# metacraft-labs/dvt-circuits

Hardware: AMD Instinct MI355X
Metric: SP1 prover cycles/sec + proofs/hour, finalization_prove at 1/2/4/8 MI355X (higher is better)
Workload: dtype u32; 1 GPU; BASELINE configs[1] input: examples/finalization_test.json (tests/golden/finalization_example.json) through the reference's JSON -> CBOR -> SP1Stdin encoding, executed AND proven (the whole prove() call) by the finalization-shaped synthetic guest tests/guests.py:dkg_like(6180, 1545, 1): 32 shards of 2^21 RV32IM cycles; the reference's own guest ELF is prebuilt machine code and is not run (it would; stdin_bytes=2165, participants=3, curve_precompiles=False, fri_queries=100, pow_bits=16, log_blowup=1

## Files before the change

### dvt_circuits_amd/capi.py

```python
import ctypes as C
import json
import os
import subprocess

import numpy as np

HERE = os.path.dirname(os.path.abspath(__file__))
LIB_PATH = os.path.join(HERE, "libdvt_prover.so")
CSRC = os.path.join(HERE, "csrc")

DVT_OK, DVT_ERR_GUEST, DVT_ERR_INPUT, DVT_ERR_DEVICE, DVT_ERR_UNSUPPORTED, DVT_ERR_REJECTED = 0, 1, 2, 3, 4, 5
PATHS = {"default": 0, "rows": 1, "parts": 2}
SELECTORS = {"table": 0, "kernel": 1}
DVT_KEEP_NONE, DVT_KEEP_TREE, DVT_KEEP_FULL = 0, 1, 2
u32p = C.POINTER(C.c_uint32)
u8p = C.POINTER(C.c_uint8)


class DevMatrix(C.Structure):
    _fields_ = [("d_data", C.c_void_p), ("width", C.c_uint32), ("log_height", C.c_uint32)]


class HostTrace(C.Structure):
    _fields_ = [("chip_id", C.c_uint32), ("log_n", C.c_uint32), ("data", u32p)]
# ... 86 lines not shown
    lib.dvt_stage_hunt_join_free.argtypes = [vp, vp]
    lib.dvt_rv32_hunt_join_job.argtypes = [vp, vp, vp, C.POINTER(JoinWindow), sz, u32p, u32, u64, u32p, u32, u32p, u32p, u64, sz, sz, u32,
                                           C.POINTER(JoinSummary), C.POINTER(JoinCell), sz, C.POINTER(sz), C.POINTER(JoinCell), sz, C.POINTER(sz)]
    lib.dvt_rv32_job_shard_chips.argtypes = [vp, sz]
    lib.dvt_rv32_job_shard_chips.restype = u32
    lib.dvt_rv32_job_shard_chip_shape.argtypes = [vp, sz, u32, u32p, u32p]
    lib.dvt_machine_setup.argtypes = [vp, C.c_char_p, C.POINTER(HostTrace), sz, C.POINTER(vp), C.POINTER(u8p), C.POINTER(sz)]
    lib.dvt_pk_free.argtypes = [vp, vp]
    lib.dvt_pk_free.restype = None
    lib.dvt_machine_prove.argtypes = [vp, vp, C.POINTER(HostTrace), sz, u32p, sz, C.POINTER(u8p), C.POINTER(sz)]
    lib.dvt_machine_verify.argtypes = [C.c_char_p, sz, C.c_char_p, sz, u32, u32, C.POINTER(C.c_char_p)]
    lib.dvt_prover_machine_verify.argtypes = [vp, C.c_char_p, sz, C.c_char_p, sz, u32, u32, C.POINTER(C.c_char_p)]
    lib.dvt_prover_verify.argtypes = [vp, C.c_char_p, sz, C.c_char_p, sz, u32, u32, C.POINTER(C.c_int32), C.POINTER(u8p), C.POINTER(sz), C.POINTER(C.c_char_p)]
    lib.dvt_prover_verify_times.argtypes = [vp, C.POINTER(C.c_double)]
    lib.dvt_stage_sponge_rows.argtypes = [vp, u32p, u32p, sz, u32p]
    lib.dvt_stage_verify_paths.argtypes = [vp, C.POINTER(PathChain), sz, u8p]
    lib.dvt_stage_multipath_nodes.argtypes = [u32, u32p, sz, u32p, sz, C.POINTER(sz)]
    lib.dvt_stage_verify_multipath.argtypes = [vp, u32, u32p, u32p, sz, u8p, u32p, u32p, sz, u32p, u8p]
    for fn in (lib.dvt_proof_compact, lib.dvt_proof_expand):
        fn.argtypes = [C.c_char_p, sz, C.c_char_p, sz, u32, u32, C.POINTER(u8p), C.POINTER(sz), C.POINTER(C.c_char_p)]
    lib.dvt_debug_compact_list_sweep.argtypes = [C.c_char_p, sz, C.c_char_p, sz, u32, u32, C.POINTER(u64), C.POINTER(u64), C.POINTER(C.c_char_p)]
    lib.dvt_last_stage_ms.argtypes = [vp, C.POINTER(C.c_float)]
    lib.dvt_setup.argtypes = [vp, C.c_char_p, sz, C.POINTER(vp), C.POINTER(u8p), C.POINTER(sz)]
    lib.dvt_execute.argtypes = [C.c_char_p, sz, C.POINTER(Buf), sz, C.c_uint64, C.POINTER(u8p), C.POINTER(sz), C.POINTER(Report), C.POINTER(C.c_char_p)]
    lib.dvt_execute_io.argtypes = [C.c_char_p, sz, C.POINTER(Buf), sz, C.c_uint64, C.POINTER(u8p), C.POINTER(sz), C.POINTER(u8p), C.POINTER(sz), C.POINTER(Report), C.POINTER(C.c_char_p)]
    lib.dvt_debug_exec_rate.argtypes = [C.c_char_p, sz, C.POINTER(Buf), sz, u32, C.c_int]
    lib.dvt_debug_exec_rate.restype = C.c_double
    lib.dvt_debug_p2_f64_selfcheck.argtypes = [u32, u32]
    lib.dvt_debug_p2_f64_selfcheck.restype = u64
    lib.dvt_debug_p2_f64_sbox_check.argtypes = [u32, u32, C.POINTER(C.c_double)]
    lib.dvt_debug_p2_f64_sbox_check.restype = u64
    lib.dvt_debug_ntt_group_check.argtypes = [u32, u32] + [C.POINTER(C.c_double)] * 3
    lib.dvt_debug_ntt_group_check.restype = u64
    lib.dvt_prove_core.argtypes = [vp, vp, C.POINTER(Buf), sz, C.POINTER(u8p), C.POINTER(sz), C.POINTER(Report)]
    lib.dvt_verify.argtypes = [C.c_char_p, sz, C.c_char_p, sz, u32, u32, C.POINTER(C.c_int32), C.POINTER(u8p), C.POINTER(sz), C.POINTER(C.c_char_p)]
    lib.dvt_rv32_prepare.argtypes = [vp, vp, C.POINTER(Buf), sz, C.POINTER(vp), C.POINTER(Report)]
    lib.dvt_rv32_prepare_part.argtypes = [vp, vp, C.POINTER(Buf), sz, sz, sz, C.POINTER(vp), C.POINTER(Report)]
    lib.dvt_rv32_header_words.restype = u32
    lib.dvt_rv32_job_exec_wait_seconds.argtypes = [vp]
    lib.dvt_rv32_job_exec_wait_seconds.restype = C.c_double
    lib.dvt_rv32_prove_job.argtypes = [vp, vp, vp, C.POINTER(u8p), C.POINTER(sz)]
    lib.dvt_job_free.argtypes = [vp, vp]
    lib.dvt_job_free.restype = None
    lib.dvt_rv32_debug_traces.argtypes = [C.c_char_p, sz, C.POINTER(Buf), sz, u32, u32, u32p, C.POINTER(u32p), C.POINTER(sz), C.POINTER(C.c_char_p)]
    lib.dvt_rv32_job_shards.argtypes = [vp]
    lib.dvt_rv32_job_shards.restype = sz
    lib.dvt_rv32_job_shard_member.argtypes = [vp, sz]
    lib.dvt_rv32_job_shard_member.restype = C.c_int
    lib.dvt_rv32_job_shard_device_rows.argtypes = [vp, sz]
    lib.dvt_rv32_job_shard_device_rows.restype = u32
    lib.dvt_rv32_job_shard_kept.argtypes = [vp, sz]
    lib.dvt_rv32_job_shard_kept.restype = C.c_int
    lib.dvt_rv32_job_shard_kept_bytes.argtypes = [vp, sz]
    lib.dvt_rv32_job_shard_kept_bytes.restype = C.c_uint64
    lib.dvt_debug_keep_plan.argtypes = [C.c_int, u64, u64, u64, u64, u64, u64, u64, C.c_int, C.c_int64, u64]
    lib.dvt_debug_keep_plan.restype = C.c_int
    lib.dvt_rv32_commit_shard.argtypes = [vp, vp, vp, sz, u32p]
    lib.dvt_rv32_challenges.argtypes = [C.c_char_p, sz, u32p, sz, u32p]
    lib.dvt_rv32_prove_shard.argtypes = [vp, vp, vp, sz, u32p, C.POINTER(u8p), C.POINTER(sz)]
    lib.dvt_rv32_assemble.argtypes = [vp, C.POINTER(C.c_char_p), C.POINTER(sz), sz, C.POINTER(u8p), C.POINTER(sz)]
    lib.dvt_rv32_debug_device_traces.argtypes = [vp, vp, vp, sz, C.POINTER(u32p), C.POINTER(sz)]
    lib.dvt_rv32_debug_poke_cell.argtypes = [vp, vp, sz, u32, u32, u32, u32]
    prof_out = [C.POINTER(u64), sz, C.POINTER(ProfileEdge), sz, C.POINTER(ProfileSyscall), sz, C.POINTER(ProfileOpcode), sz, C.POINTER(ProfileSummary)]
    lib.dvt_rv32_job_profile.argtypes = [vp, vp, vp, u32] + prof_out
    lib.dvt_execute_profile.argtypes = [C.c_char_p, sz, C.POINTER(Buf), sz, u64] + prof_out + [C.POINTER(Report), C.POINTER(C.c_char_p)]
    tree_out = [C.POINTER(CalltreeArc), sz, C.POINTER(CalltreeFunc), sz, C.POINTER(CalltreeSummary)]
# ... 629 lines not shown
                    max_cycles=0, log_shard=21):
    lib = load()
    reps, err = (Report(), Report()), C.c_char_p()
    a, b = bytes(stdin_a), bytes(stdin_b)
    rc, got = _diverge(lambda *io: lib.dvt_execute_diverge(elf, len(elf), a, len(a), b, len(b), max_cycles, log_shard, *io, C.byref(reps[0]), C.byref(reps[1]),
                                                           C.byref(err)), start_a, start_b, max_pairs, rejoin, window, keep)
    return rc, tuple(dict(cycles=r.cycles, exit_code=r.exit_code, halted=bool(r.halted), unprovable=bool(r.unprovable)) for r in reps), got, _take_str(lib, err)


def exec_rate(elf: bytes, stdin=(), log_shard=21, trace=False) -> float:
    return float(load().dvt_debug_exec_rate(elf, len(elf), _bufs(stdin), len(stdin), log_shard, int(trace)))


def keep_plan(mode, free, total, reserve, full, tree, later, remaining=0, count_known=True, full_cap=-1, full_kept=0) -> int:
    return int(load().dvt_debug_keep_plan(mode, free, total, reserve, full, tree, later, remaining, int(bool(count_known)), full_cap, full_kept))


def p2_f64_selfcheck(n: int, seed: int) -> int:
    return int(load().dvt_debug_p2_f64_selfcheck(n, seed))


def p2_f64_sbox_check(n: int, seed: int):
    mx = (C.c_double * 4)()
    bad = load().dvt_debug_p2_f64_sbox_check(n, seed, mx)
    return int(bad), [float(v) for v in mx]


def ntt_group_check(n: int, seed: int):
    mx = [(C.c_double * 8)() for _ in range(3)]
    bad = load().dvt_debug_ntt_group_check(n, seed, *mx)
    return int(bad), {k: [float(v) for v in m] for k, m in zip(("dif", "dif_unit", "dit"), mx)}


def execute_io(elf: bytes, stdin=(), max_cycles=0):
    lib = load()
    pv, n, so, m, rep, err = u8p(), C.c_size_t(), u8p(), C.c_size_t(), Report(), C.c_char_p()
    rc = lib.dvt_execute_io(elf, len(elf), _bufs(stdin), len(stdin), max_cycles, C.byref(pv), C.byref(n), C.byref(so), C.byref(m), C.byref(rep), C.byref(err))
    out = C.string_at(pv, n.value) if pv else b""
    sout = C.string_at(so, m.value) if so else b""
    for ptr in (pv, so):
        if ptr:
            lib.dvt_free(C.cast(ptr, C.c_void_p))
    return rc, dict(cycles=rep.cycles, exit_code=rep.exit_code, halted=bool(rep.halted), unprovable=bool(rep.unprovable)), out, sout, _take_str(lib, err)


def stdin_from_json(circuit_type: str, json_bytes: bytes, auth_commitment=False) -> bytes:
    lib = load()
    out, n, err = u8p(), C.c_size_t(), C.c_char_p()
    rc = lib.dvt_stdin_from_json(circuit_type.encode(), json_bytes, len(json_bytes), int(bool(auth_commitment)), C.byref(out), C.byref(n), C.byref(err))
    if rc:
        raise DvtError(rc, _take_str(lib, err))
    b = C.string_at(out, n.value)
    lib.dvt_free(C.cast(out, C.c_void_p))
    return b


def verify(vk: bytes, proof: bytes, fri_queries=100, pow_bits=16):
    lib = load()
    ec, pv, n, why = C.c_int32(), u8p(), C.c_size_t(), C.c_char_p()
    rc = lib.dvt_verify(vk, len(vk), proof, len(proof), fri_queries, pow_bits, C.byref(ec), C.byref(pv), C.byref(n), C.byref(why))
    out = C.string_at(pv, n.value) if pv else b""
    if pv:
        lib.dvt_free(C.cast(pv, C.c_void_p))
    return rc == DVT_OK, ec.value, out, _take_str(lib, why)


# ... 658 lines not shown
```

### dvt_circuits_amd/csrc/bb.cuh

```cuda
#pragma once
#include <stdint.h>

#if defined(__HIPCC__)
#include <hip/hip_runtime.h>
#if defined(__HIP_DEVICE_COMPILE__)
#define DVT_HD __host__ __device__ __forceinline__
#else
#define DVT_HD __host__ __device__ inline
#endif
#else
#define DVT_HD inline
#endif

namespace dvt {

constexpr uint32_t P = 0x78000001u;
constexpr uint32_t MONTY_MU = 0x88000001u;
constexpr uint32_t MONTY_R = 0x0ffffffeu;
constexpr uint32_t MONTY_R2 = 0x45dddde3u;
static_assert((uint32_t)(P * MONTY_MU) == 1u, "mu");
static_assert(((uint64_t)1 << 32) % P == MONTY_R, "R");
static_assert((((uint64_t)MONTY_R * MONTY_R) % P) == MONTY_R2, "R2");

DVT_HD uint32_t mulhi_u32(uint32_t a, uint32_t b) {
// ... 67 lines not shown
    Fp c[4];
    DVT_HD static Fp4 zero() { Fp4 r; r.c[0] = r.c[1] = r.c[2] = r.c[3] = Fp::zero(); return r; }
    DVT_HD static Fp4 one() { Fp4 r = zero(); r.c[0] = Fp::one(); return r; }
    DVT_HD static Fp4 from_base(Fp a) { Fp4 r = zero(); r.c[0] = a; return r; }
    DVT_HD bool operator==(const Fp4 &o) const { return c[0] == o.c[0] && c[1] == o.c[1] && c[2] == o.c[2] && c[3] == o.c[3]; }
    DVT_HD bool operator!=(const Fp4 &o) const { return !(*this == o); }
};
DVT_HD Fp mul11(Fp a) {
    Fp a2 = dbl(a), a4 = dbl(a2), a8 = dbl(a4);
    return a8 + a2 + a;
}
DVT_HD Fp4 operator+(const Fp4 &a, const Fp4 &b) { Fp4 r; for (int i = 0; i < 4; i++) r.c[i] = a.c[i] + b.c[i]; return r; }
DVT_HD Fp4 operator-(const Fp4 &a, const Fp4 &b) { Fp4 r; for (int i = 0; i < 4; i++) r.c[i] = a.c[i] - b.c[i]; return r; }
DVT_HD Fp4 operator-(const Fp4 &a) { Fp4 r; for (int i = 0; i < 4; i++) r.c[i] = -a.c[i]; return r; }
DVT_HD Fp4 operator+(const Fp4 &a, Fp b) { Fp4 r = a; r.c[0] = r.c[0] + b; return r; }
DVT_HD Fp4 operator-(const Fp4 &a, Fp b) { Fp4 r = a; r.c[0] = r.c[0] - b; return r; }
DVT_HD Fp4 operator*(const Fp4 &a, Fp b) { Fp4 r; for (int i = 0; i < 4; i++) r.c[i] = a.c[i] * b; return r; }
DVT_HD Fp4 operator*(const Fp4 &a, const Fp4 &b) {
    Fp4 r;
    r.c[0] = a.c[0] * b.c[0] + mul11(a.c[1] * b.c[3] + a.c[2] * b.c[2] + a.c[3] * b.c[1]);
    r.c[1] = a.c[0] * b.c[1] + a.c[1] * b.c[0] + mul11(a.c[2] * b.c[3] + a.c[3] * b.c[2]);
    r.c[2] = a.c[0] * b.c[2] + a.c[1] * b.c[1] + a.c[2] * b.c[0] + mul11(a.c[3] * b.c[3]);
    r.c[3] = a.c[0] * b.c[3] + a.c[1] * b.c[2] + a.c[2] * b.c[1] + a.c[3] * b.c[0];
    return r;
}
DVT_HD Fp4 &operator+=(Fp4 &a, const Fp4 &b) { a = a + b; return a; }
DVT_HD Fp4 &operator-=(Fp4 &a, const Fp4 &b) { a = a - b; return a; }
DVT_HD Fp4 &operator*=(Fp4 &a, const Fp4 &b) { a = a * b; return a; }
DVT_HD Fp4 pow(Fp4 a, uint64_t e) {
    Fp4 r = Fp4::one();
    while (e) { if (e & 1) r = r * a; a = a * a; e >>= 1; }
    return r;
}
DVT_HD Fp4 inv(const Fp4 &a) {
    Fp A0 = a.c[0], A1 = a.c[2], B0 = a.c[1], B1 = a.c[3];
    Fp A2_0 = A0 * A0 + mul11(A1 * A1), A2_1 = dbl(A0 * A1);
    Fp B2_0 = B0 * B0 + mul11(B1 * B1), B2_1 = dbl(B0 * B1);
    Fp D0 = A2_0 - mul11(B2_1), D1 = A2_1 - B2_0;
    Fp ni = inv(D0 * D0 - mul11(D1 * D1));
    Fp I0 = D0 * ni, I1 = -(D1 * ni);
    Fp4 r;
    r.c[0] = A0 * I0 + mul11(A1 * I1);
    r.c[2] = A0 * I1 + A1 * I0;
    r.c[1] = -(B0 * I0 + mul11(B1 * I1));
    r.c[3] = -(B0 * I1 + B1 * I0);
    return r;
}

}
```

### dvt_circuits_amd/csrc/capi_rv32.hip

```cpp
#include <algorithm>
#include <atomic>
#include <cstdio>
#include <deque>
#include <map>

#include "capi_job.h"
#include "ntt_group.cuh"
#include "poseidon2_f64.cuh"
#include "sha256.h"

using namespace dvt;
static_assert(DVT_KEEP_NONE == KEEP_NONE && DVT_KEEP_TREE == KEEP_TREE && DVT_KEEP_FULL == KEEP_FULL, "the tiers of include/dvt_prover.h");

namespace {
std::vector<std::vector<uint8_t>> collect_stdin(const dvt_buf *bufs, size_t n) {
    std::vector<std::vector<uint8_t>> v(n);
    for (size_t i = 0; i < n; i++)
        if (bufs[i].len) v[i].assign(bufs[i].data, bufs[i].data + bufs[i].len);
    return v;
}
uint8_t *dup_bytes(const std::vector<uint8_t> &v, size_t *len) {
    uint8_t *b = (uint8_t *)malloc(v.size() + 1);
    if (b && !v.empty()) memcpy(b, v.data(), v.size());
    if (len) *len = v.size();
// ... 1541 lines not shown
uint64_t dvt_debug_ntt_group_check(uint32_t n, uint32_t seed, double *max_dif, double *max_dif_unit, double *max_dit) {
    uint64_t bad = 0, s = 0x9e3779b97f4a7c15ull ^ seed;
    double mx[3][8] = {};
    const int64_t lim[3] = {(int64_t)ntg::DIF_IN, (int64_t)ntg::DIF_IN, (int64_t)ntg::DIT_IN}, half = ((int64_t)P - 1) / 2;
    auto next = [&]() { s ^= s << 13; s ^= s >> 7; s ^= s << 17; return s; };
    auto uniform = [&](int64_t m) { return (int64_t)(next() % (2 * (uint64_t)m + 1)) - m; };
    int64_t in[8], tw[7];
    for (uint32_t g = 0; g < n; g++)
        for (int kind = 0; kind < 3; kind++) {
            for (int j = 0; j < 8; j++) in[j] = uniform(lim[kind]);
            for (int k = 0; k < 7; k++) tw[k] = uniform(half);
            bad += ntg_check_one(kind, in, tw, mx[kind]);
        }
    const int64_t mags[5] = {0, 1, half, (int64_t)P - 1, (int64_t)(0.52 * p2f::PD)};
    const int64_t tws[4] = {1, -1, half, -half};
    for (int kind = 0; kind < 3; kind++)
        for (int m = 0; m < 5; m++)
            for (int signs = 0; signs < 256; signs++) {
                if (m == 0 && signs) break;
                const int64_t mag = mags[m] > lim[kind] ? lim[kind] : mags[m];
                for (int j = 0; j < 8; j++) in[j] = (signs >> j) & 1 ? -mag : mag;
                for (int c = 0; c < 64 + 8; c++) {
                    for (int k = 0; k < 7; k++) {
                        const int stage = kind == 2 ? (k < 1 ? 0 : k < 3 ? 1 : 2) : (k < 4 ? 0 : k < 6 ? 1 : 2);
                        tw[k] = c < 64 ? tws[(c >> (2 * stage)) & 3] : uniform(half);
                    }
                    bad += ntg_check_one(kind, in, tw, mx[kind]);
                }
            }
    for (int k = 0; k < 8; k++) { max_dif[k] = mx[0][k]; max_dif_unit[k] = mx[1][k]; max_dit[k] = mx[2][k]; }
    return bad;
}

}
```

### dvt_circuits_amd/csrc/fri.hip

```cpp
#include "kernels.h"
#include "poseidon2_f64.cuh"
#include "f64dot.cuh"

namespace dvt {

__device__ __forceinline__ Fp root_pow24f(const NttTables &t, uint32_t e) {
    return Fp::raw(t.tw_hi[e >> 12]) * Fp::raw(t.tw_lo[e & 4095]);
}
__device__ __forceinline__ Fp4 load_ext(const Fp4 *p) {
    uint4 v = *reinterpret_cast<const uint4 *>(p);
    Fp4 r;
    r.c[0] = Fp::raw(v.x); r.c[1] = Fp::raw(v.y); r.c[2] = Fp::raw(v.z); r.c[3] = Fp::raw(v.w);
    return r;
}
__device__ __forceinline__ void store_ext(Fp4 *p, const Fp4 &v) {
    *reinterpret_cast<uint4 *>(p) = make_uint4(v.c[0].v, v.c[1].v, v.c[2].v, v.c[3].v);
}

constexpr int SCAN_PER_THREAD = 8, SCAN_BLOCK = 256 * SCAN_PER_THREAD;

__global__ void __launch_bounds__(256) scan_blocks_kernel(uint32_t *data, size_t n, uint32_t *block_sums, size_t nblocks) {
    __shared__ uint32_t wsum[256];
    uint32_t *col = data + (size_t)blockIdx.y * n;
    size_t base = (size_t)blockIdx.x * SCAN_BLOCK + (size_t)threadIdx.x * SCAN_PER_THREAD;
// ... 37 lines not shown
hipError_t launch_prefix_sum_columns(hipStream_t st, uint32_t *d_cols, uint32_t ncols, size_t n, uint32_t *d_scratch) {
    size_t nblocks = (n + SCAN_BLOCK - 1) / SCAN_BLOCK;
    dim3 grid((unsigned)nblocks, ncols);
    scan_blocks_kernel<<<grid, 256, 0, st>>>(d_cols, n, d_scratch, nblocks);
    if (nblocks > 1) {
        scan_sums_kernel<<<1, ncols, 0, st>>>(d_scratch, nblocks);
        scan_add_kernel<<<grid, 256, 0, st>>>(d_cols, n, d_scratch, nblocks);
    }
    return hipGetLastError();
}
size_t prefix_sum_scratch_words(uint32_t ncols, size_t n) { return ncols * ((n + SCAN_BLOCK - 1) / SCAN_BLOCK); }

__global__ void __launch_bounds__(256) phi_from_prefix_sums_kernel(const uint32_t *tot, uint32_t *phi, size_t n, Fp n_inv, uint32_t *cum_out) {
    size_t r = (size_t)blockIdx.x * blockDim.x + threadIdx.x;
    if (r >= n) return;
    if (r == n - 1 && cum_out) {
#pragma unroll
        for (int k = 0; k < 4; k++) cum_out[k] = tot[(size_t)k * n + n - 1];
    }
    const Fp rf = Fp::from_canonical((uint32_t)r) * n_inv;
#pragma unroll
    for (int k = 0; k < 4; k++) {
        const Fp c = Fp::raw(tot[(size_t)k * n + n - 1]) * rf;
        const Fp before = r ? Fp::raw(tot[(size_t)k * n + r - 1]) : Fp::zero();
        phi[(size_t)k * n + r] = (before - c).v;
    }
}
hipError_t launch_phi_from_prefix_sums(hipStream_t st, const uint32_t *d_totals, uint32_t *d_phi, uint32_t log_n, uint32_t *cum_out) {
    const size_t n = (size_t)1 << log_n;
    phi_from_prefix_sums_kernel<<<(unsigned)((n + 255) / 256), 256, 0, st>>>(d_totals, d_phi, n, inv(Fp::from_canonical((uint32_t)n)), cum_out);
    return hipGetLastError();
}

__global__ void __launch_bounds__(256) open_weights_kernel(Fp4 z, uint32_t log_n, Fp4 *w, NttTables tabs) {
    size_t i = (size_t)blockIdx.x * blockDim.x + threadIdx.x;
    if (i >= ((size_t)1 << log_n)) return;
    Fp x = root_pow24f(tabs, (uint32_t)i << (24 - log_n));
    Fp4 d = z - x;
    Fp4 r = inv(d) * x;
#pragma unroll
    for (int k = 0; k < 4; k++) {
        const uint32_t c = r.c[k].canonical();
        r.c[k] = Fp::raw(c > P / 2 ? c - P : c);
    }
    store_ext(w + i, r);
}
hipError_t launch_open_weights(hipStream_t st, const NttTables &tabs, Fp4 z, uint32_t log_n, Fp4 *d_w) {
    size_t n = (size_t)1 << log_n;
    open_weights_kernel<<<(unsigned)((n + 255) / 256), 256, 0, st>>>(z, log_n, d_w, tabs);
    return hipGetLastError();
}

constexpr int OPEN_CT = 4;
__global__ void __launch_bounds__(256) open_columns_kernel(const uint32_t *const *cols, uint32_t ncols, uint32_t log_n,
                                                          const Fp4 *w, Fp4 *partial) {
    __shared__ uint32_t red[256 * 4];
    const size_t n = (size_t)1 << log_n;
    const uint32_t c0 = blockIdx.y * OPEN_CT;
    DotAcc acc_l[OPEN_CT][4], acc_n[OPEN_CT][4];
#pragma unroll
    for (int c = 0; c < OPEN_CT; c++)
#pragma unroll
        for (int k = 0; k < 4; k++) acc_l[c][k] = acc_n[c][k] = DotAcc{0.0, 0.0};
    const size_t stride = (size_t)gridDim.x * 256;
    size_t i = (size_t)blockIdx.x * 256 + threadIdx.x;
    Fp4 wl, wn;
    uint32_t v[OPEN_CT];
    auto fetch = [&](size_t row) {
        wl = load_ext(w + row);
        wn = load_ext(w + ((row + n - 1) & (n - 1)));
#pragma unroll
        for (int c = 0; c < OPEN_CT; c++) v[c] = c0 + c < ncols ? cols[c0 + c][row] : 0u;
    };
    if (i < n) fetch(i);
    for (uint32_t it = 0; i < n; i += stride, it++) {
        double dl[4], dn[4], vlo[OPEN_CT], vhi[OPEN_CT];
#pragma unroll
        for (int k = 0; k < 4; k++) { dl[k] = (double)(int32_t)wl.c[k].v; dn[k] = (double)(int32_t)wn.c[k].v; }
#pragma unroll
        for (int c = 0; c < OPEN_CT; c++) { vlo[c] = (double)(v[c] & 0xffffu); vhi[c] = (double)(v[c] >> 16); }
        if (i + stride < n) fetch(i + stride);
#pragma unroll
// ... 74 lines not shown
            uint32_t v[8];
#pragma unroll
            for (int u = 0; u < 8; u++) v[u] = a.cols[c + u][i];
#pragma unroll
            for (int u = 0; u < 8; u++) {
                const double vlo = (double)(v[u] & 0xffffu), vhi = (double)(v[u] >> 16);
#pragma unroll
                for (int k = 0; k < 4; k++) acc[k].add(a.alpha_pows[4 * (c + u) + k], vlo, vhi);
            }
            if (((c - from) & 8) != 0)
#pragma unroll
                for (int k = 0; k < 4; k++) acc[k].reduce();
        }
#pragma unroll
        for (int k = 0; k < 4; k++) acc[k].reduce();
        for (; c < to; c++) {
            const uint32_t v = a.cols[c][i];
            const double vlo = (double)(v & 0xffffu), vhi = (double)(v >> 16);
#pragma unroll
            for (int k = 0; k < 4; k++) acc[k].add(a.alpha_pows[4 * c + k], vlo, vhi);
        }
#pragma unroll
        for (int k = 0; k < 4; k++) acc[k].reduce();
    };
    sweep(0, a.n_two);
#pragma unroll
    for (int k = 0; k < 4; k++) s_two.c[k] = acc[k].value();
    sweep(a.n_two, a.n_all);
    Fp4 s;
#pragma unroll
    for (int k = 0; k < 4; k++) s.c[k] = acc[k].value();
    if (a.n_two == a.n_all) s_two = s;
    Fp x = Fp::raw(a.tabs.sh_lo[1]) * root_pow24f(a.tabs, (uint32_t)i << (24 - a.log_m));
    Fp4 r = (s - a.sz_all) * inv(Fp4::from_base(x) - a.zeta);
    if (a.n_two) r += a.alpha_shift * ((s_two - a.sz_two) * inv(Fp4::from_base(x) - a.zeta_next));
    store_ext(a.out + i, r);
}
hipError_t launch_reduced_opening(hipStream_t st, const NttTables &tabs, const uint32_t *const *d_cols, uint32_t n_two,
                                  uint32_t n_all, uint32_t log_m, const double *d_alpha_pows_f64, Fp4 sz_all, Fp4 sz_two, Fp4 zeta,
                                  Fp4 zeta_next, Fp4 alpha_shift, Fp4 *d_out) {
    ReducedArgs a{d_cols, n_two, n_all, log_m, d_alpha_pows_f64, sz_all, sz_two, zeta, zeta_next, alpha_shift, d_out, tabs};
    size_t m = (size_t)1 << log_m;
    reduced_opening_kernel<<<(unsigned)((m + 255) / 256), 256, 0, st>>>(a);
    return hipGetLastError();
}

__global__ void __launch_bounds__(256) fri_fold_kernel(const Fp4 *v, Fp4 *out, const Fp4 *ro, Fp4 beta, const Fp4 *beta_dev,
                                                      uint32_t log_m, Fp inv2, NttTables tabs) {
    const size_t half = (size_t)1 << (log_m - 1);
    size_t i = (size_t)blockIdx.x * blockDim.x + threadIdx.x;
    if (i >= half) return;
    if (beta_dev) beta = load_ext(beta_dev);
    Fp4 lo = load_ext(v + i), hi = load_ext(v + i + half);
    Fp xinv = i ? root_pow24f(tabs, (uint32_t)(2 * half - i) << (24 - log_m)) : Fp::one();
    Fp4 r = (lo + hi) * inv2 + beta * ((lo - hi) * (inv2 * xinv));
    if (ro) r += load_ext(ro + i);
    store_ext(out + i, r);
}
hipError_t launch_fri_fold(hipStream_t st, const NttTables &tabs, const Fp4 *d_v, Fp4 *d_out, const Fp4 *d_ro, Fp4 beta,
                           uint32_t log_m, const Fp4 *d_beta) {
    size_t half = (size_t)1 << (log_m - 1);
    Fp inv2 = inv(Fp::two());
    fri_fold_kernel<<<(unsigned)((half + 255) / 256), 256, 0, st>>>(d_v, d_out, d_ro, beta, d_beta, log_m, inv2, tabs);
    return hipGetLastError();
}
__global__ void __launch_bounds__(64) fri_challenge_kernel(const uint32_t *root, uint32_t *state, Fp4 *beta_out, uint32_t *root_out) {
    const uint32_t e = threadIdx.x & 15;
    const p2f::CoopConsts k = p2f::coop_consts(e);
// ... 111 lines not shown
```

### dvt_circuits_amd/csrc/kernels.h

```cpp
#pragma once
#include <hip/hip_runtime.h>

#include <algorithm>
#include <cstddef>
#include <cstdint>
#include <vector>

#include "bb.cuh"
#include "poseidon2.cuh"

namespace dvt {

constexpr uint32_t LDE_MAX_LOG = 23;
struct NttTables {
    uint32_t *base = nullptr;
    const uint32_t *tw_hi = nullptr, *tw_lo = nullptr, *sh_hi = nullptr, *sh_lo = nullptr;
    const uint32_t *lde_tw = nullptr, *lde_scale = nullptr;
    const uint32_t *lde_tw_c = nullptr, *lde_scale_c = nullptr;
};
hipError_t ntt_tables_create(NttTables *t);
void ntt_tables_destroy(NttTables *t);

hipError_t launch_coset_lde(hipStream_t st, const NttTables &tabs, uint32_t *d_in, uint32_t *d_scratch, uint32_t *d_out,
                            uint32_t width, uint32_t log_n, uint32_t shift_mode);
hipError_t launch_to_internal(hipStream_t st, uint32_t *d, size_t n);
hipError_t launch_from_internal(hipStream_t st, uint32_t *d, size_t n);

constexpr uint32_t MERKLE_TOP_LOG = 6;
constexpr uint32_t MERKLE_COOP_LOG = 13;
constexpr uint32_t MERKLE_MAX_SEGMENTS = 24;
struct MerkleLeafSegments {
    uint32_t n = 0;
    const uint32_t *const *cols[MERKLE_MAX_SEGMENTS];
    uint32_t *out[MERKLE_MAX_SEGMENTS];
    uint32_t ncols[MERKLE_MAX_SEGMENTS], log_h[MERKLE_MAX_SEGMENTS];
    uint32_t coop[MERKLE_MAX_SEGMENTS];
    uint32_t block0[MERKLE_MAX_SEGMENTS + 1];
    void add(const uint32_t *const *c, uint32_t nc, uint32_t lh, uint32_t *o) { cols[n] = c; ncols[n] = nc; log_h[n] = lh; out[n] = o; n++; }
};
hipError_t launch_merkle_leaves(hipStream_t st, MerkleLeafSegments sg);
hipError_t launch_merkle_level(hipStream_t st, const uint32_t *d_prev, const uint32_t *d_inject, uint32_t log_len, uint32_t *d_out);
struct MerkleTopInject {
    const uint32_t *digests[MERKLE_TOP_LOG + 1] = {};
};
hipError_t launch_merkle_top(hipStream_t st, uint32_t *d_layer, uint32_t log_start, const MerkleTopInject &inj);
hipError_t launch_poseidon2_permute(hipStream_t st, uint32_t *d_states, size_t n);

hipError_t launch_prefix_sum_columns(hipStream_t st, uint32_t *d_cols, uint32_t ncols, size_t n, uint32_t *d_scratch);
size_t prefix_sum_scratch_words(uint32_t ncols, size_t n);
hipError_t launch_phi_from_prefix_sums(hipStream_t st, const uint32_t *d_totals, uint32_t *d_phi, uint32_t log_n, uint32_t *cum_out);
hipError_t launch_open_weights(hipStream_t st, const NttTables &tabs, Fp4 z, uint32_t log_n, Fp4 *d_w);
constexpr uint32_t OPEN_MAX_ROW_BLOCKS = 256;
uint32_t open_row_blocks(uint32_t log_n);
hipError_t launch_open_columns(hipStream_t st, const uint32_t *const *d_cols, uint32_t ncols, uint32_t log_n, const Fp4 *d_w,
                               Fp4 *d_partial, Fp4 *d_out);
hipError_t launch_reduced_opening(hipStream_t st, const NttTables &tabs, const uint32_t *const *d_cols, uint32_t n_two,
                                  uint32_t n_all, uint32_t log_m, const double *d_alpha_pows_f64, Fp4 sz_all, Fp4 sz_two, Fp4 zeta,
                                  Fp4 zeta_next, Fp4 alpha_shift, Fp4 *d_out);
hipError_t launch_fri_fold(hipStream_t st, const NttTables &tabs, const Fp4 *d_v, Fp4 *d_out, const Fp4 *d_ro, Fp4 beta,
                           uint32_t log_m, const Fp4 *d_beta = nullptr);
hipError_t launch_fri_challenge(hipStream_t st, const uint32_t *d_root, uint32_t *d_state, Fp4 *d_beta_out, uint32_t *d_root_out);
hipError_t launch_fri_leaves(hipStream_t st, const Fp4 *d_v, uint32_t log_m, uint32_t *d_digests);
hipError_t launch_gather_rows(hipStream_t st, const uint32_t *const *d_cols, const uint32_t *d_log_h, uint32_t ncols,
                              const uint32_t *d_idx, uint32_t nq, uint32_t *d_out);
hipError_t launch_gather_paths(hipStream_t st, const uint32_t *d_digests, uint32_t log_h, const uint32_t *d_idx, uint32_t nq,
                               uint32_t *d_out);
hipError_t launch_gather_nodes(hipStream_t st, const uint32_t *d_digests, const uint32_t *d_at, uint32_t n, uint32_t *d_out);
hipError_t launch_gather_siblings(hipStream_t st, const Fp4 *d_v, uint32_t log_m, const uint32_t *d_idx, uint32_t nq, Fp4 *d_out);
hipError_t launch_pow_grind(hipStream_t st, const uint32_t state[16], uint32_t pos, uint32_t bits, uint32_t base, uint32_t count,
                            uint32_t *d_found);


namespace rv32 { struct CycleRec; }
enum ProfileCounter { PROFILE_TRANSFERS, PROFILE_DROPPED, PROFILE_SYS_OVERFLOW, PROFILE_BAD_RECORDS, PROFILE_COUNTERS };
struct ProfileTables {
    unsigned long long *pc_count, *taken;
    unsigned long long *edge_keys, *edge_counts;
    unsigned long long *sys_keys, *sys_counts;
    unsigned long long *counters;
    const uint32_t *classes;
    uint32_t n_instr, log_slots;
};
hipError_t launch_profile_records(hipStream_t st, const rv32::CycleRec *d_recs, size_t n_recs, uint32_t last_succ, const ProfileTables &t);
// ... 87 lines not shown
```

### dvt_circuits_amd/csrc/machine_rv32.hip

```cpp
#include "machine.h"
#if !defined(__HIP_DEVICE_COMPILE__)
#pragma clang optimize off
#endif
#include "gen/air_rv32.inc"
#if !defined(__HIP_DEVICE_COMPILE__)
#pragma clang optimize on
#endif

namespace dvt {
ChipDesc rv32_wide_chip_desc(int chip);
void rv32_check_fns(int chip, ChipDesc *d);
void rv32_wide_check_fns(int chip, ChipDesc *d);
void rv32_ledger_fns(int chip, ChipDesc *d);
void rv32_wide_ledger_fns(int chip, ChipDesc *d);
void rv32_hunt_fns(int chip, ChipDesc *d);
void rv32_wide_hunt_fns(int chip, ChipDesc *d);
void rv32_join_fns(int chip, ChipDesc *d);
void rv32_wide_join_fns(int chip, ChipDesc *d);
namespace {
template <int I, class A>
ChipDesc chip_desc_here() {
    ChipDesc d;
    if constexpr (I < RV32_FIRST_WIDE_CHIP) { d = make_chip_desc<A>(); rv32_check_fns(I, &d); rv32_ledger_fns(I, &d); rv32_hunt_fns(I, &d); rv32_join_fns(I, &d); }
    else { d = rv32_wide_chip_desc(I); rv32_wide_check_fns(I, &d); rv32_wide_ledger_fns(I, &d); rv32_wide_hunt_fns(I, &d); rv32_wide_join_fns(I, &d); }
    return d;
}
}
#define DVT_X(i, A) chip_desc_here<i, A>(),
static const ChipDesc rv32_chips[] = {DVT_AIR_RV32_CHIPS(DVT_X)};
#undef DVT_X
static const MachineDesc rv32_machine = {"rv32", air_rv32::N_CHIPS, rv32_chips};
const MachineDesc *machine_rv32() { return &rv32_machine; }
}
```

### dvt_circuits_amd/csrc/stark.cuh

```cuda
#pragma once
#include "bb.cuh"
#include "f64dot.cuh"
#include "kernels.h"

namespace dvt {

constexpr int WHEN_ALL = 0, WHEN_FIRST = 1, WHEN_LAST = 2, WHEN_TRANS = 3;

DVT_HD Fp4 to_ext(Fp a) { return Fp4::from_base(a); }
DVT_HD Fp4 to_ext(const Fp4 &a) { return a; }

template <class Air>
struct PermShape {
    static constexpr int NB = (Air::N_INTERACTIONS + 1) / 2;
    static constexpr int EXT_W = Air::N_INTERACTIONS ? NB : 0;
    static constexpr int PHI = NB - 1;
    static constexpr int BASE_W = 4 * EXT_W;
    static constexpr int N_FOLDED = Air::N_CONSTRAINTS + (Air::N_INTERACTIONS ? NB : 0);
};

template <class Air, class TT, class Access>
struct ConstraintFolder {
    using T = TT;
    using Shape = PermShape<Air>;
// ... 147 lines not shown
            Air::interactions(*this);
        } else if constexpr (PART < Air::N_PARTS) {
            Air::template constraints_part<PART>(*this);
        } else {
            Air::template interactions_part<PART - Air::N_PARTS>(*this);
        }
        if constexpr (BASE) {
            acc += acc_d.value();
            Fp4 lc;
            for (int k = 0; k < 4; k++) lc.c[k] = Fp::raw(p2f::to_mont(acc_c.c[k]));
            acc += lc;
        }
        return acc;
    }
};

#if defined(__HIPCC__)
struct PermArgs {
    const uint32_t *main;
    const uint32_t *prep;
    const uint32_t *pub;
    uint32_t *perm;
    uint32_t *totals;
    const Fp4 *beta_pows;
    const double *beta_d;
    Fp4 perm_alpha;
    uint32_t log_n;
    uint32_t *partial = nullptr;
};
constexpr int PARTS_MAX = 32;
constexpr uint32_t PARTS_PARALLEL_LOG = 15;

template <class Air>
struct PermRowCtx {
    using T = Fp;
    const PermArgs &a;
    size_t n, row;
    Fp4 batch, total;
    __device__ PermRowCtx(const PermArgs &args, size_t r) : a(args), n((size_t)1 << args.log_n), row(r), batch(Fp4::zero()), total(Fp4::zero()) {}
    __device__ static T K(uint32_t m) { return Fp::raw(m); }
    __device__ static T KI(uint32_t canonical) { return Fp::from_canonical(canonical); }
    __device__ T main(int c, int r) const { return Fp::raw(a.main[(size_t)c * n + ((row + r) & (n - 1))]); }
    __device__ T prep(int c, int r) const { return Fp::raw(a.prep[(size_t)c * n + ((row + r) & (n - 1))]); }
    __device__ T pub(int k) const { return Fp::raw(a.pub[k]); }
    __device__ void store_ext(int extcol, const Fp4 &v) {
#pragma unroll
        for (int k = 0; k < 4; k++) a.perm[((size_t)(4 * extcol + k)) * n + row] = v.c[k].v;
    }
    __device__ void interaction(int j, int bus, int sign, int , const T &mult, const T *vals, int nv) {
        Fp4 term = Fp4::zero();
        if (!mult.is_zero()) {
            DotAcc4 s;
            for (int k = 0; k < nv; k++) {
                s.add(a.beta_d + 4 * k, vals[k]);
                if ((k & 31) == 31) s.reduce();
            }
            Fp4 d = a.perm_alpha + Fp::from_canonical((uint32_t)bus) + s.value();
            term = inv(d) * (sign > 0 ? mult : -mult);
        }
        if ((j & 1) == 0) batch = term; else batch += term;
        if ((j & 1) || j == Air::N_INTERACTIONS - 1) {
            if ((j >> 1) < PermShape<Air>::PHI) store_ext(j >> 1, batch);
            total += batch;
        }
    }
};

template <class Air>
__global__ void __launch_bounds__(256) perm_rows_kernel(PermArgs a) {
    size_t row = (size_t)blockIdx.x * blockDim.x + threadIdx.x;
    if (row >= ((size_t)1 << a.log_n)) return;
    PermRowCtx<Air> ctx(a, row);
    Air::interactions(ctx);
#pragma unroll
    for (int k = 0; k < 4; k++) a.totals[(size_t)k * ctx.n + row] = ctx.total.c[k].v;
}

template <class Air, int LP, class Ctx>
__device__ __forceinline__ void interactions_of_part(Ctx &ctx, int part) {
    if (part == LP) Air::template interactions_part<LP>(ctx);
    else if constexpr (LP + 1 < Air::N_LPARTS) interactions_of_part<Air, LP + 1>(ctx, part);
}
template <class Air>
__global__ void __launch_bounds__(256) perm_rows_parts_kernel(PermArgs a) {
    size_t row = (size_t)blockIdx.x * blockDim.x + threadIdx.x;
    if (row >= ((size_t)1 << a.log_n)) return;
    PermRowCtx<Air> ctx(a, row);
    interactions_of_part<Air, 0>(ctx, (int)blockIdx.y);
#pragma unroll
    for (int k = 0; k < 4; k++) a.partial[((size_t)blockIdx.y * 4 + k) * ctx.n + row] = ctx.total.c[k].v;
}
template <int UNUSED>
__global__ void __launch_bounds__(256) sum_parts_kernel(const uint32_t *partial, uint32_t nparts, size_t words, uint32_t *out) {
    size_t w = (size_t)blockIdx.x * blockDim.x + threadIdx.x;
    if (w >= words) return;
    Fp acc = Fp::raw(partial[w]);
    for (uint32_t p = 1; p < nparts; p++) acc = acc + Fp::raw(partial[(size_t)p * words + w]);
    out[w] = acc.v;
}

struct QuotientArgs {
    const uint32_t *main_lde;
    const uint32_t *prep_lde;
    const uint32_t *perm_lde;
    const uint32_t *pub;
    uint32_t *out;
    const Fp4 *alpha_pows;
    const Fp4 *beta_pows;
    const double *alpha_d, *beta_d;
    Fp4 perm_alpha, cum_over_n;
    Fp zinv_even, zinv_odd;
    Fp z_even, z_odd;
    Fp w_inv;
    uint32_t log_n;
    NttTables tabs;
    const uint32_t *sel = nullptr;
    uint32_t *partial = nullptr;
};

__device__ __forceinline__ void selectors_of_row(const QuotientArgs &a, size_t i, Fp *sel_first, Fp *sel_last, Fp *sel_trans) {
    const uint32_t log_m = a.log_n + 1;
// ... 100 lines not shown
```

### include/dvt_prover.h

```cpp
#ifndef DVT_PROVER_H
#define DVT_PROVER_H
#include <stddef.h>
#include <stdint.h>
#ifdef __cplusplus
extern "C" {
#endif

#define DVT_OK 0
#define DVT_ERR_GUEST 1
#define DVT_ERR_INPUT 2
#define DVT_ERR_DEVICE 3
#define DVT_ERR_UNSUPPORTED 4
#define DVT_ERR_REJECTED 5

typedef struct dvt_prover dvt_prover;
typedef struct dvt_pk dvt_pk;

int dvt_prover_create(const char *cfg_json, dvt_prover **out);
uint32_t dvt_prover_device_count(const dvt_prover *p);
int dvt_prover_device(const dvt_prover *p, uint32_t member);
void dvt_prover_destroy(dvt_prover *p);
const char *dvt_last_error(const dvt_prover *p);
void dvt_free(void *ptr);
uint32_t dvt_abi_version(void);
// ... 406 lines not shown
} dvt_diverge_summary;
int dvt_rv32_job_diverge(dvt_prover *p, const dvt_pk *pk, dvt_job *job_a, dvt_job *job_b, dvt_diverge_pos start_a, dvt_diverge_pos start_b,
                         uint64_t max_pairs, uint32_t flags, uint32_t window, size_t cap_each, dvt_diverge_pair *first, dvt_diverge_pair *last,
                         dvt_diverge_reg regs[32], dvt_diverge_summary *summary);
int dvt_rv32_job_diverge_times(dvt_prover *p, double out[4]);
int dvt_execute_diverge(const uint8_t *elf, size_t elf_len, const uint8_t *stdin_a, size_t n_a, const uint8_t *stdin_b, size_t n_b, uint64_t max_cycles,
                        uint32_t log_shard_size, dvt_diverge_pos start_a, dvt_diverge_pos start_b, uint64_t max_pairs, uint32_t flags, uint32_t window,
                        size_t cap_each, dvt_diverge_pair *first, dvt_diverge_pair *last, dvt_diverge_reg regs[32], dvt_diverge_summary *summary,
                        dvt_report *report_a, dvt_report *report_b, char **err_text);
int dvt_rv32_debug_device_traces(dvt_prover *p, const dvt_pk *pk, dvt_job *job, size_t shard, uint32_t **blob,
                                 size_t *blob_words);
int dvt_rv32_debug_poke_cell(dvt_prover *p, dvt_job *job, size_t shard, uint32_t chip, uint32_t col, uint32_t row,
                             uint32_t add);
int dvt_verify(const uint8_t *vk, size_t vk_len, const uint8_t *proof, size_t proof_len, uint32_t fri_queries,
               uint32_t pow_bits, int32_t *exit_code, uint8_t **public_values, size_t *pv_len, char **reason);
int dvt_prover_verify(dvt_prover *p, const uint8_t *vk, size_t vk_len, const uint8_t *proof, size_t proof_len,
                      uint32_t fri_queries, uint32_t pow_bits, int32_t *exit_code, uint8_t **public_values,
                      size_t *pv_len, char **reason);
int dvt_proof_compact(const uint8_t *vk, size_t vk_len, const uint8_t *proof, size_t proof_len, uint32_t fri_queries,
                      uint32_t pow_bits, uint8_t **out, size_t *out_len, char **reason);
int dvt_proof_expand(const uint8_t *vk, size_t vk_len, const uint8_t *proof, size_t proof_len, uint32_t fri_queries,
                     uint32_t pow_bits, uint8_t **out, size_t *out_len, char **reason);
int dvt_debug_compact_list_sweep(const uint8_t *vk, size_t vk_len, const uint8_t *proof, size_t proof_len, uint32_t fri_queries,
                                 uint32_t pow_bits, uint64_t *n_words, uint64_t *n_accepted, char **reason);
int dvt_prover_verify_times(dvt_prover *p, double out[9]);
int dvt_debug_keep_plan(int mode, uint64_t free_bytes, uint64_t total_bytes, uint64_t reserve_bytes, uint64_t full_bytes,
                        uint64_t tree_bytes, uint64_t later_bytes, uint64_t remaining, int count_known, int64_t full_cap,
                        uint64_t full_kept);
double dvt_debug_exec_rate(const uint8_t *elf, size_t elf_len, const dvt_buf *stdin_bufs, size_t nbuf, uint32_t log_shard,
                           int trace);
uint64_t dvt_debug_p2_f64_selfcheck(uint32_t n, uint32_t seed);
uint64_t dvt_debug_p2_f64_sbox_check(uint32_t n, uint32_t seed, double *max_abs);
uint64_t dvt_debug_ntt_group_check(uint32_t n, uint32_t seed, double *max_dif, double *max_dif_unit, double *max_dit);
uint64_t dvt_debug_ledger_key(uint64_t seed, uint32_t bus, uint32_t arity, const uint32_t *values);

int dvt_stdin_from_json(const char *type, const char *json, size_t json_len, int auth_commitment, uint8_t **out,
                        size_t *out_len, char **err_text);
int dvt_json_schema_validate(const char *schema, size_t schema_len, const char *json, size_t json_len, char **err_text);

int dvt_rv32_debug_traces(const uint8_t *elf, size_t elf_len, const dvt_buf *stdin_bufs, size_t nbuf, uint32_t log_shard,
                          uint32_t shard, uint32_t *n_shards, uint32_t **blob, size_t *blob_words, char **err_text);

#ifdef __cplusplus
}
#endif
#endif
```

Baseline: 82.15 million guest cycles/s.

## Share one base-field inversion across groups of Fp4 denominators

Adds a Montgomery batch-inversion helper for quartic-extension elements, built on the norm/conjugate split of the Fp4 inverse. It is used in the permutation trace rows (groups of 8 for the CPU chip, 2 elsewhere), in FRI open weights (4 points per thread) and in the reduced opening's two denominators. The aim is to replace several costly base-field exponentiation inversions with one inversion plus a few extra multiplications. In exchange it raises register pressure from the per-row arrays, which may lower occupancy, and it adds debug self-check entry points.

New measurement: 82.36 million guest cycles/s (median of 2 runs). Within noise of the previous version (+0.3%).

```diff
diff --git a/dvt_circuits_amd/capi.py b/dvt_circuits_amd/capi.py
--- a/dvt_circuits_amd/capi.py
+++ b/dvt_circuits_amd/capi.py
@@ -142,6 +142,8 @@
     lib.dvt_debug_p2_f64_sbox_check.restype = u64
     lib.dvt_debug_ntt_group_check.argtypes = [u32, u32] + [C.POINTER(C.c_double)] * 3
     lib.dvt_debug_ntt_group_check.restype = u64
+    lib.dvt_debug_k4_group_size.restype = u32
+    lib.dvt_debug_fp4_shared_inverse.argtypes = [u32, u32p, u8p, u32p, u32p]
     lib.dvt_prove_core.argtypes = [vp, vp, C.POINTER(Buf), sz, C.POINTER(u8p), C.POINTER(sz), C.POINTER(Report)]
     lib.dvt_verify.argtypes = [C.c_char_p, sz, C.c_char_p, sz, u32, u32, C.POINTER(C.c_int32), C.POINTER(u8p), C.POINTER(sz), C.POINTER(C.c_char_p)]
     lib.dvt_rv32_prepare.argtypes = [vp, vp, C.POINTER(Buf), sz, C.POINTER(vp), C.POINTER(Report)]
@@ -837,6 +839,23 @@
     return int(bad), {k: [float(v) for v in m] for k, m in zip(("dif", "dif_unit", "dit"), mx)}
 
 
+def k4_group_size() -> int:
+    return int(load().dvt_debug_k4_group_size())
+
+
+def fp4_shared_inverse(den, live):
+    g = len(den)
+    flat = [int(w) for d in den for w in d]
+    a = (C.c_uint32 * (4 * g))(*flat)
+    lv = (C.c_uint8 * g)(*[1 if x else 0 for x in live])
+    shared, direct = (C.c_uint32 * (4 * g))(), (C.c_uint32 * (4 * g))()
+    rc = load().dvt_debug_fp4_shared_inverse(g, a, lv, shared, direct)
+    if rc != DVT_OK:
+        raise DvtError(rc, f"dvt_debug_fp4_shared_inverse({g})")
+    rows = lambda t: [[int(t[4 * i + k]) for k in range(4)] for i in range(g)]
+    return rows(shared), rows(direct)
+
+
 def execute_io(elf: bytes, stdin=(), max_cycles=0):
     lib = load()
     pv, n, so, m, rep, err = u8p(), C.c_size_t(), u8p(), C.c_size_t(), Report(), C.c_char_p()
diff --git a/dvt_circuits_amd/csrc/bb.cuh b/dvt_circuits_amd/csrc/bb.cuh
--- a/dvt_circuits_amd/csrc/bb.cuh
+++ b/dvt_circuits_amd/csrc/bb.cuh
@@ -123,13 +123,16 @@
     while (e) { if (e & 1) r = r * a; a = a * a; e >>= 1; }
     return r;
 }
-DVT_HD Fp4 inv(const Fp4 &a) {
+DVT_HD Fp fp4_norm(const Fp4 &a, Fp *D0, Fp *D1) {
     Fp A0 = a.c[0], A1 = a.c[2], B0 = a.c[1], B1 = a.c[3];
     Fp A2_0 = A0 * A0 + mul11(A1 * A1), A2_1 = dbl(A0 * A1);
     Fp B2_0 = B0 * B0 + mul11(B1 * B1), B2_1 = dbl(B0 * B1);
-    Fp D0 = A2_0 - mul11(B2_1), D1 = A2_1 - B2_0;
-    Fp ni = inv(D0 * D0 - mul11(D1 * D1));
-    Fp I0 = D0 * ni, I1 = -(D1 * ni);
+    *D0 = A2_0 - mul11(B2_1); *D1 = A2_1 - B2_0;
+    return *D0 * *D0 - mul11(*D1 * *D1);
+}
+DVT_HD Fp4 fp4_conj_times(const Fp4 &a, Fp D0, Fp D1, Fp s) {
+    Fp A0 = a.c[0], A1 = a.c[2], B0 = a.c[1], B1 = a.c[3];
+    Fp I0 = D0 * s, I1 = -(D1 * s);
     Fp4 r;
     r.c[0] = A0 * I0 + mul11(A1 * I1);
     r.c[2] = A0 * I1 + A1 * I0;
@@ -137,5 +140,37 @@
     r.c[3] = -(B0 * I1 + B1 * I0);
     return r;
 }
+DVT_HD Fp4 inv(const Fp4 &a) {
+    Fp D0, D1;
+    const Fp n = fp4_norm(a, &D0, &D1);
+    return fp4_conj_times(a, D0, D1, inv(n));
+}
+
+template <int G>
+DVT_HD void inv_shared(const Fp4 *d, const bool *live, Fp4 *out, const Fp *scale = nullptr) {
+    Fp D0[G], D1[G], nrm[G], before[G];
+    Fp run = Fp::one();
+    bool any = false;
+#pragma unroll
+    for (int g = 0; g < G; g++)
+        if (live[g]) {
+            const Fp n = fp4_norm(d[g], &D0[g], &D1[g]);
+            nrm[g] = n.is_zero() ? Fp::one() : n;
+            before[g] = run;
+            run = run * nrm[g];
+            any = true;
+        }
+    if (any) run = inv(run);
+#pragma unroll
+    for (int g = G - 1; g >= 0; g--) {
+        out[g] = Fp4::zero();
+        if (live[g]) {
+            Fp s = run * before[g];
+            run = run * nrm[g];
+            if (scale) s = s * scale[g];
+            out[g] = fp4_conj_times(d[g], D0[g], D1[g], s);
+        }
+    }
+}
 
 }
diff --git a/dvt_circuits_amd/csrc/capi_rv32.hip b/dvt_circuits_amd/csrc/capi_rv32.hip
--- a/dvt_circuits_amd/csrc/capi_rv32.hip
+++ b/dvt_circuits_amd/csrc/capi_rv32.hip
@@ -1597,4 +1597,34 @@
     return bad;
 }
 
-}
+extern "C++" {
+template <int G>
+static void shared_inverse_both(const uint32_t *den, const uint8_t *live, uint32_t *shared, uint32_t *direct) {
+    Fp4 d[G], r[G];
+    bool lv[G];
+    for (int g = 0; g < G; g++) {
+        for (int k = 0; k < 4; k++) d[g].c[k] = Fp::raw(den[4 * g + k]);
+        lv[g] = live[g] != 0;
+    }
+    inv_shared<G>(d, lv, r);
+    for (int g = 0; g < G; g++) {
+        const Fp4 want = lv[g] ? inv(d[g]) : Fp4::zero();
+        for (int k = 0; k < 4; k++) { shared[4 * g + k] = r[g].c[k].v; direct[4 * g + k] = want.c[k].v; }
+    }
+}
+}
+uint32_t dvt_debug_k4_group_size(void) { return (uint32_t)K4_GROUP_CPU; }
+int dvt_debug_fp4_shared_inverse(uint32_t g, const uint32_t *den, const uint8_t *live, uint32_t *shared, uint32_t *direct) {
+    if (!den || !live || !shared || !direct) return DVT_ERR_INPUT;
+    if (g != 1 && g != 2 && g != 4 && g != 8 && g != (uint32_t)K4_GROUP_CPU) return DVT_ERR_INPUT;
+    for (uint32_t k = 0; k < 4 * g; k++)
+        if (den[k] >= P) return DVT_ERR_INPUT;
+    if (g == 1) shared_inverse_both<1>(den, live, shared, direct);
+    else if (g == 2) shared_inverse_both<2>(den, live, shared, direct);
+    else if (g == 4) shared_inverse_both<4>(den, live, shared, direct);
+    else if (g == 8) shared_inverse_both<8>(den, live, shared, direct);
+    else shared_inverse_both<K4_GROUP_CPU>(den, live, shared, direct);
+    return DVT_OK;
+}
+
+}
diff --git a/dvt_circuits_amd/csrc/fri.hip b/dvt_circuits_amd/csrc/fri.hip
--- a/dvt_circuits_amd/csrc/fri.hip
+++ b/dvt_circuits_amd/csrc/fri.hip
@@ -93,22 +93,35 @@
     return hipGetLastError();
 }
 
+template <int R>
 __global__ void __launch_bounds__(256) open_weights_kernel(Fp4 z, uint32_t log_n, Fp4 *w, NttTables tabs) {
+    const size_t per = ((size_t)1 << log_n) / R;
     size_t i = (size_t)blockIdx.x * blockDim.x + threadIdx.x;
-    if (i >= ((size_t)1 << log_n)) return;
-    Fp x = root_pow24f(tabs, (uint32_t)i << (24 - log_n));
-    Fp4 d = z - x;
-    Fp4 r = inv(d) * x;
-#pragma unroll
-    for (int k = 0; k < 4; k++) {
-        const uint32_t c = r.c[k].canonical();
-        r.c[k] = Fp::raw(c > P / 2 ? c - P : c);
-    }
-    store_ext(w + i, r);
+    if (i >= per) return;
+    Fp x[R];
+    Fp4 d[R], r[R];
+    bool live[R];
+#pragma unroll
+    for (int q = 0; q < R; q++) {
+        x[q] = root_pow24f(tabs, (uint32_t)(i + q * per) << (24 - log_n));
+        d[q] = z - x[q];
+        live[q] = true;
+    }
+    inv_shared<R>(d, live, r, x);
+#pragma unroll
+    for (int q = 0; q < R; q++) {
+#pragma unroll
+        for (int k = 0; k < 4; k++) {
+            const uint32_t c = r[q].c[k].canonical();
+            r[q].c[k] = Fp::raw(c > P / 2 ? c - P : c);
+        }
+        store_ext(w + i + q * per, r[q]);
+    }
 }
 hipError_t launch_open_weights(hipStream_t st, const NttTables &tabs, Fp4 z, uint32_t log_n, Fp4 *d_w) {
     size_t n = (size_t)1 << log_n;
-    open_weights_kernel<<<(unsigned)((n + 255) / 256), 256, 0, st>>>(z, log_n, d_w, tabs);
+    if (log_n >= 2) open_weights_kernel<4><<<(unsigned)((n / 4 + 255) / 256), 256, 0, st>>>(z, log_n, d_w, tabs);
+    else open_weights_kernel<1><<<1, 256, 0, st>>>(z, log_n, d_w, tabs);
     return hipGetLastError();
 }
 
@@ -249,8 +262,12 @@
     for (int k = 0; k < 4; k++) s.c[k] = acc[k].value();
     if (a.n_two == a.n_all) s_two = s;
     Fp x = Fp::raw(a.tabs.sh_lo[1]) * root_pow24f(a.tabs, (uint32_t)i << (24 - a.log_m));
-    Fp4 r = (s - a.sz_all) * inv(Fp4::from_base(x) - a.zeta);
-    if (a.n_two) r += a.alpha_shift * ((s_two - a.sz_two) * inv(Fp4::from_base(x) - a.zeta_next));
+    const Fp4 den[2] = {Fp4::from_base(x) - a.zeta, Fp4::from_base(x) - a.zeta_next};
+    const bool live[2] = {true, a.n_two != 0};
+    Fp4 di[2];
+    inv_shared<2>(den, live, di);
+    Fp4 r = (s - a.sz_all) * di[0];
+    if (a.n_two) r += a.alpha_shift * ((s_two - a.sz_two) * di[1]);
     store_ext(a.out + i, r);
 }
 hipError_t launch_reduced_opening(hipStream_t st, const NttTables &tabs, const uint32_t *const *d_cols, uint32_t n_two,
diff --git a/dvt_circuits_amd/csrc/kernels.h b/dvt_circuits_amd/csrc/kernels.h
--- a/dvt_circuits_amd/csrc/kernels.h
+++ b/dvt_circuits_amd/csrc/kernels.h
@@ -49,6 +49,7 @@
 hipError_t launch_prefix_sum_columns(hipStream_t st, uint32_t *d_cols, uint32_t ncols, size_t n, uint32_t *d_scratch);
 size_t prefix_sum_scratch_words(uint32_t ncols, size_t n);
 hipError_t launch_phi_from_prefix_sums(hipStream_t st, const uint32_t *d_totals, uint32_t *d_phi, uint32_t log_n, uint32_t *cum_out);
+constexpr int K4_GROUP_CPU = 8;
 hipError_t launch_open_weights(hipStream_t st, const NttTables &tabs, Fp4 z, uint32_t log_n, Fp4 *d_w);
 constexpr uint32_t OPEN_MAX_ROW_BLOCKS = 256;
 uint32_t open_row_blocks(uint32_t log_n);
diff --git a/dvt_circuits_amd/csrc/machine_rv32.hip b/dvt_circuits_amd/csrc/machine_rv32.hip
--- a/dvt_circuits_amd/csrc/machine_rv32.hip
+++ b/dvt_circuits_amd/csrc/machine_rv32.hip
@@ -8,6 +8,10 @@
 #endif
 
 namespace dvt {
+template <>
+struct PermGroup<air_rv32::Cpu> {
+    static constexpr int G = K4_GROUP_CPU;
+};
 ChipDesc rv32_wide_chip_desc(int chip);
 void rv32_check_fns(int chip, ChipDesc *d);
 void rv32_wide_check_fns(int chip, ChipDesc *d);
diff --git a/dvt_circuits_amd/csrc/stark.cuh b/dvt_circuits_amd/csrc/stark.cuh
--- a/dvt_circuits_amd/csrc/stark.cuh
+++ b/dvt_circuits_amd/csrc/stark.cuh
@@ -203,12 +203,22 @@
 constexpr uint32_t PARTS_PARALLEL_LOG = 15;
 
 template <class Air>
+struct PermGroup {
+    static constexpr int G = 2;
+};
+
+template <class Air>
 struct PermRowCtx {
     using T = Fp;
+    static constexpr int G = PermGroup<Air>::G;
+    static_assert(G >= 2 && G % 2 == 0, "a group is whole batch columns");
     const PermArgs &a;
     size_t n, row;
-    Fp4 batch, total;
-    __device__ PermRowCtx(const PermArgs &args, size_t r) : a(args), n((size_t)1 << args.log_n), row(r), batch(Fp4::zero()), total(Fp4::zero()) {}
+    Fp4 total;
+    Fp4 den[G];
+    Fp mul[G];
+    int first = 0, cnt = 0;
+    __device__ PermRowCtx(const PermArgs &args, size_t r) : a(args), n((size_t)1 << args.log_n), row(r), total(Fp4::zero()) {}
     __device__ static T K(uint32_t m) { return Fp::raw(m); }
     __device__ static T KI(uint32_t canonical) { return Fp::from_canonical(canonical); }
     __device__ T main(int c, int r) const { return Fp::raw(a.main[(size_t)c * n + ((row + r) & (n - 1))]); }
@@ -218,22 +228,43 @@
 #pragma unroll
         for (int k = 0; k < 4; k++) a.perm[((size_t)(4 * extcol + k)) * n + row] = v.c[k].v;
     }
-    __device__ void interaction(int j, int bus, int sign, int , const T &mult, const T *vals, int nv) {
-        Fp4 term = Fp4::zero();
+    template <int S = 0>
+    __device__ __forceinline__ void put(int slot, const Fp4 &d, Fp m) {
+        if (slot == S) { den[S] = d; mul[S] = m; }
+        else if constexpr (S + 1 < G) put<S + 1>(slot, d, m);
+    }
+    __device__ __forceinline__ void flush() {
+        bool live[G];
+        Fp4 term[G];
+#pragma unroll
+        for (int s = 0; s < G; s++) live[s] = s < cnt && !mul[s].is_zero();
+        inv_shared<G>(den, live, term, mul);
+#pragma unroll
+        for (int k = 0; k < G / 2; k++)
+            if (2 * k < cnt) {
+                const Fp4 batch = term[2 * k] + term[2 * k + 1];
+                if (first / 2 + k < PermShape<Air>::PHI) store_ext(first / 2 + k, batch);
+                total += batch;
+            }
+        cnt = 0;
+    }
+    __device__ __forceinline__ void interaction(int j, int bus, int sign, int , const T &mult, const T *vals, int nv) {
+        Fp4 d = Fp4::zero();
         if (!mult.is_zero()) {
             DotAcc4 s;
             for (int k = 0; k < nv; k++) {
                 s.add(a.beta_d + 4 * k, vals[k]);
                 if ((k & 31) == 31) s.reduce();
             }
-            Fp4 d = a.perm_alpha + Fp::from_canonical((uint32_t)bus) + s.value();
-            term = inv(d) * (sign > 0 ? mult : -mult);
-        }
-        if ((j & 1) == 0) batch = term; else batch += term;
-        if ((j & 1) || j == Air::N_INTERACTIONS - 1) {
-            if ((j >> 1) < PermShape<Air>::PHI) store_ext(j >> 1, batch);
-            total += batch;
-        }
+            d = a.perm_alpha + Fp::from_canonical((uint32_t)bus) + s.value();
+        }
+        if (cnt == 0) first = j;
+        put(cnt++, d, sign > 0 ? mult : -mult);
+        if (cnt == G || j == Air::N_INTERACTIONS - 1) flush();
+    }
+    __device__ __forceinline__ void finish() {
+        if constexpr (G > 2)
+            if (cnt) flush();
     }
 };
 
@@ -243,6 +274,7 @@
     if (row >= ((size_t)1 << a.log_n)) return;
     PermRowCtx<Air> ctx(a, row);
     Air::interactions(ctx);
+    ctx.finish();
 #pragma unroll
     for (int k = 0; k < 4; k++) a.totals[(size_t)k * ctx.n + row] = ctx.total.c[k].v;
 }
@@ -258,6 +290,7 @@
     if (row >= ((size_t)1 << a.log_n)) return;
     PermRowCtx<Air> ctx(a, row);
     interactions_of_part<Air, 0>(ctx, (int)blockIdx.y);
+    ctx.finish();
 #pragma unroll
     for (int k = 0; k < 4; k++) a.partial[((size_t)blockIdx.y * 4 + k) * ctx.n + row] = ctx.total.c[k].v;
 }
diff --git a/include/dvt_prover.h b/include/dvt_prover.h
--- a/include/dvt_prover.h
+++ b/include/dvt_prover.h
@@ -462,6 +462,8 @@
 uint64_t dvt_debug_p2_f64_selfcheck(uint32_t n, uint32_t seed);
 uint64_t dvt_debug_p2_f64_sbox_check(uint32_t n, uint32_t seed, double *max_abs);
 uint64_t dvt_debug_ntt_group_check(uint32_t n, uint32_t seed, double *max_dif, double *max_dif_unit, double *max_dit);
+uint32_t dvt_debug_k4_group_size(void);
+int dvt_debug_fp4_shared_inverse(uint32_t g, const uint32_t *den, const uint8_t *live, uint32_t *shared, uint32_t *direct);
 uint64_t dvt_debug_ledger_key(uint64_t seed, uint32_t bus, uint32_t arity, const uint32_t *values);
 
 int dvt_stdin_from_json(const char *type, const char *json, size_t json_len, int auth_commitment, uint8_t **out,
```
